# embedded-software-laboratory/p-dmpc

Hardware: AMD Instinct MI355X
Metric: MPC steps/sec (whole node) + p50 per-step plan latency, N vehicles H=8 (higher is better)
Workload: dtype f64

## Files before the change

include/pdmpc.h:

```cpp
#ifndef PDMPC_H
#define PDMPC_H

#include <stddef.h>
#include <stdint.h>

#ifdef __cplusplus
extern "C" {
#endif

#define PDMPC_HP_MAX 16
#define PDMPC_VMAX 8
#define PDMPC_JOINT_MAX 4

enum {
    PDMPC_OK = 0,
    PDMPC_EXHAUSTED = 1,
    PDMPC_ARENA_OVERFLOW = 2,
    PDMPC_ERR_INVALID = -1,
    PDMPC_ERR_NO_DEVICE = -2,
    PDMPC_ERR_HIP = -3,
    PDMPC_ERR_CAPACITY = -4,
    PDMPC_ERR_NO_MPA = -5
};

// ... 114 lines not shown
    uint32_t bk_near_key, bk_near_id, bk_ready, bk_hist, bk_misc, bk_pshape, reach_shared, bk_reach, reach;
    uint32_t ints, succ, heap_key, heap_id;
    const char* kernel;
} pdmpc_launch_plan;
int pdmpc_launch_plan_host(const char* tuning, const pdmpc_launch_query* query, pdmpc_launch_plan* plan);

int pdmpc_get_config(pdmpc_handle* handle, pdmpc_config* config, int32_t* mpa_uploaded);

int pdmpc_upload_mpa(pdmpc_handle* handle, const pdmpc_mpa* mpa);
int pdmpc_mpa_reach_host(const pdmpc_mpa* mpa, double* dmax, double* amax);
int pdmpc_reach_lists_host(int32_t Hp, double dmax, double amax, double root_x, double root_y, const double* x, const double* y, const int32_t* step_first,
                           const int32_t* step_count, int32_t* list_offset, int32_t* list);
int pdmpc_mpa_reach_rects_host(const pdmpc_mpa* mpa, int32_t Hp, double* rects);
int pdmpc_reach_lists_oriented_host(int32_t Hp, int32_t n_trims, const double* rects, int32_t root_trim, double root_x, double root_y, double root_yaw, const double* x, const double* y,
                                    const int32_t* step_first, const int32_t* step_count, int32_t* list_offset, int32_t* list);

int pdmpc_plan_batch(pdmpc_handle* handle, int32_t n_vehicles, const pdmpc_vehicle_in* in,
                     pdmpc_vehicle_out* out);

int pdmpc_set_arena_limit(pdmpc_handle* handle, int32_t max_nodes_limit);
int pdmpc_grow_arena(pdmpc_handle* handle, int32_t max_nodes);
int pdmpc_arena_nodes(pdmpc_handle* handle, int32_t* max_nodes, int64_t* regrows);

int pdmpc_plan_step(pdmpc_handle* handle, int32_t n_vehicles, const pdmpc_vehicle_in* in, const int32_t* pred_offset,
                    const int32_t* pred_index, const pdmpc_polygon_set* fallback_shapes, pdmpc_vehicle_out* out);

int pdmpc_plan_step_literal(pdmpc_handle* handle, int32_t n_vehicles, const pdmpc_vehicle_in* in, const int32_t* pred_offset, const int32_t* pred_index,
                            const pdmpc_polygon_set* fallback_shapes, pdmpc_vehicle_out* out);

int pdmpc_pack_batch(pdmpc_handle* handle, int32_t n_vehicles, const pdmpc_vehicle_in* in);
// ... 44 lines not shown

int pdmpc_debug_pop_trace(pdmpc_handle* handle, int32_t vehicle, int32_t capacity, int32_t* ids, int32_t* n);
int pdmpc_debug_tree(pdmpc_handle* handle, int32_t vehicle, int32_t capacity, double* x, double* y,
                     double* yaw, double* g, double* h, int32_t* trim, int32_t* k, int32_t* parent,
                     int32_t* n);

int pdmpc_debug_edge_check(pdmpc_handle* handle, int32_t mode, int32_t n_cases, const int32_t* a_off, const double* a_x, const double* a_y,
                           const int32_t* b_off, const double* b_x, const double* b_y, int32_t* hit);
int pdmpc_debug_interx_soups(pdmpc_handle* handle, int32_t n_cases, const int32_t* a_off, const double* a_x, const double* a_y, const double* b_x,
                             const double* b_y, const int32_t* s_off, const double* s_x, const double* s_y, int32_t* hit);
int pdmpc_debug_sincos(pdmpc_handle* handle, int32_t n, const double* x, double* s, double* c);

int pdmpc_debug_raw_tree(pdmpc_handle* handle, int32_t vehicle, int32_t capacity, double* x, double* y, double* yaw, double* g,
                         double* h, int32_t* trim, int32_t* k, int32_t* parent, double* key, uint8_t* validity, int32_t* n);

int pdmpc_debug_counters(pdmpc_handle* handle, uint64_t* out16);
int pdmpc_debug_packed_offsets(pdmpc_handle* handle, int32_t vehicle, int32_t* lit_off, int32_t* hdv_off, int32_t* ll2);

int pdmpc_debug_progress(pdmpc_handle* handle, int32_t vehicle, uint32_t* words16);

int pdmpc_debug_heap_script(pdmpc_handle* handle, int32_t n, const int32_t* op, const int32_t* id, const double* key,
                            int32_t lds_entries, int32_t* popped, int32_t* n_popped, double* cycles_per_pop,
                            double* cycles_per_push);

int pdmpc_plan_batch_sampled(pdmpc_handle* handle, int32_t n_vehicles, const pdmpc_vehicle_in* in, const uint32_t* seeds,
                             pdmpc_vehicle_out* out);
int pdmpc_plan_step_sampled(pdmpc_handle* handle, int32_t n_vehicles, const pdmpc_vehicle_in* in, const int32_t* pred_offset,
                            const int32_t* pred_index, const pdmpc_polygon_set* fallback_shapes, const uint32_t* seeds,
                            pdmpc_vehicle_out* out);
int pdmpc_set_step_seeds(pdmpc_handle* handle, int32_t n_vehicles, const uint32_t* seeds);
int pdmpc_debug_random_numbers(pdmpc_handle* handle, int32_t count, const uint32_t* seeds, int32_t n, double* out);
// ... 240 lines not shown
```

include/pdmpc_reach.h:

```cpp
#ifndef PDMPC_REACH_H
#define PDMPC_REACH_H

#include <math.h>

#include "pdmpc_math.h"

#define PDMPC_REACH_FINITE 0x1p64
#define PDMPC_REACH_MARGIN 0x1p-20

PDMPC_HD static inline double pdmpc_reach_radius(double dmax, double amax, int k) {
    const double r = (double)(k - 1) * dmax + amax;
    return r + r * 0x1p-50;
}

PDMPC_HD static inline void pdmpc_reach_box(double dmax, double amax, int k, double root_x, double root_y, double* box) {
    const double R = pdmpc_reach_radius(dmax, amax, k);
    const double rho = R + PDMPC_REACH_MARGIN * (1.0 + fabs(root_x) + fabs(root_y) + R);
    box[0] = root_x - rho;
    box[1] = root_x + rho;
    box[2] = root_y - rho;
    box[3] = root_y + rho;
}

PDMPC_HD static inline int pdmpc_reach_in(double x0, double y0, double x1, double y1, double x_lo, double x_hi, double y_lo, double y_hi) {
// ... 19 lines not shown

PDMPC_HD static inline int pdmpc_reach_in_oriented(double x0, double y0, double x1, double y1, double root_x, double root_y, double cs, double sn, double x_lo, double x_hi, double y_lo,
                                                   double y_hi) {
    if (x0 != x0 || y0 != y0 || x1 != x1 || y1 != y1) return 0;
    const int bounded = fabs(x0) <= PDMPC_REACH_FINITE && fabs(y0) <= PDMPC_REACH_FINITE && fabs(x1) <= PDMPC_REACH_FINITE && fabs(y1) <= PDMPC_REACH_FINITE;
    if (!bounded) return 1;
    const double dx0 = x0 - root_x, dy0 = y0 - root_y, dx1 = x1 - root_x, dy1 = y1 - root_y;
    const double u0 = cs * dx0 + sn * dy0, v0 = cs * dy0 - sn * dx0;
    const double u1 = cs * dx1 + sn * dy1, v1 = cs * dy1 - sn * dx1;
    const double slack = PDMPC_REACH_ROTATION * (fabs(dx0) + fabs(dy0) + fabs(dx1) + fabs(dy1));
    const double max_u = u0 > u1 ? u0 : u1, min_u = u0 < u1 ? u0 : u1;
    const double max_v = v0 > v1 ? v0 : v1, min_v = v0 < v1 ? v0 : v1;
    return !(max_u < x_lo - slack || min_u > x_hi + slack || max_v < y_lo - slack || min_v > y_hi + slack);
}

#endif
```

p-dmpc_amd/csrc/api.cpp:

```cpp
#include <hip/hip_runtime.h>

#include <algorithm>
#include <cmath>
#include <cstdio>
#include <cstdlib>
#include <chrono>
#include <cstring>
#include <limits>
#include <mutex>
#include <string>
#include <type_traits>
#include <vector>

#include "choice_host.hpp"
#include "handle.hpp"
#include "mpa_reach.hpp"
#include "reference_tree.hpp"

namespace {

thread_local std::string g_err;

int failed(int rc, const std::string& err) { return rc ? fail(rc, err) : PDMPC_OK; }

// ... 206 lines not shown
    {
        std::string err;
        if (!parse_tuning(getenv("PDMPC_TUNING"), h->tune, err)) {
            delete h;
            return fail(PDMPC_ERR_INVALID, err);
        }
    }
    h->n_cu = prop.multiProcessorCount > 0 ? prop.multiProcessorCount : 256;
    const uint32_t want_nodes = config->max_nodes > 0 ? (uint32_t)config->max_nodes : 32768u;
    h->max_vehicles = config->max_vehicles > 0 ? config->max_vehicles : 256;
    if (hipStreamCreateWithFlags(&h->stream, hipStreamNonBlocking) != hipSuccess) {
        delete h;
        return fail(PDMPC_ERR_HIP, "hipStreamCreate failed");
    }
    int bad = h->arena.alloc(h->max_vehicles, want_nodes, h->cfg.Hp);
    bad |= h->d_out.ensure((size_t)h->max_vehicles) | h->d_flag.ensure((size_t)h->max_vehicles) | h->d_tree_size.ensure((size_t)h->max_vehicles) | h->d_tie_count.ensure(4) | h->d_work_count.ensure(16);
    bad |= h->d_help_board.ensure((size_t)h->max_vehicles * PDMPC_HB_WORDS) | h->d_help_verdict.ensure((size_t)h->max_vehicles * PDMPC_HELP_CAP) | h->d_help_finished.ensure(16);
    bad |= h->d_bk_post.ensure((size_t)h->max_vehicles * (size_t)h->tune.ready * 6);
    if (bad) {
        delete h;
        return fail(PDMPC_ERR_HIP, "hipMalloc failed for the per-vehicle arenas (lower max_nodes / max_vehicles)");
    }
    (void)hipMemsetAsync(h->d_flag.p, 0, h->d_flag.cap * sizeof(uint32_t), h->stream);
    (void)hipMemsetAsync(h->d_tree_size.p, 0, h->d_tree_size.cap * sizeof(int32_t), h->stream);
    (void)hipMemsetAsync(h->d_tie_count.p, 0, 4 * sizeof(int32_t), h->stream);
    (void)hipMemsetAsync(h->d_work_count.p, 0, 16 * sizeof(unsigned long long), h->stream);
    (void)hipMemsetAsync(h->d_out.p, 0, h->d_out.cap * sizeof(pdmpc_vehicle_out), h->stream);
    (void)hipStreamSynchronize(h->stream);
    *out_handle = h;
    return PDMPC_OK;
}

int pdmpc_launch_plan_host(const char* tuning, const pdmpc_launch_query* q, pdmpc_launch_plan* plan) {
    if (!q || !plan) return fail(PDMPC_ERR_INVALID, "pdmpc_launch_plan_host: null argument");
    if (q->kind < kPlanSearch || q->kind > kPlanJoint) return fail(PDMPC_ERR_INVALID, "pdmpc_launch_plan_host: unknown kind");
    std::string err;
    return failed(plan_query(tuning, *q, *plan, err), err);
}

int pdmpc_sampled_plan_host(const char* tuning, const pdmpc_launch_query* q, int32_t n_expansions_max, pdmpc_launch_plan* plan, int64_t* extra) {
    if (!q || !plan || !extra) return fail(PDMPC_ERR_INVALID, "pdmpc_sampled_plan_host: null argument");
// ... 96 lines not shown
}

int pdmpc_mpa_reach_rects_host(const pdmpc_mpa* mpa, int32_t Hp, double* rects) {
    if (!mpa || !rects || !mpa->transition || !mpa->maneuver_index || (mpa->n_maneuvers > 0 && !mpa->maneuvers)) return fail(PDMPC_ERR_INVALID, "pdmpc_mpa_reach_rects_host: null argument");
    if (mpa->n_trims < 1 || Hp < 1 || Hp > PDMPC_HP_MAX || Hp > mpa->Hp) return fail(PDMPC_ERR_INVALID, "pdmpc_mpa_reach_rects_host: Hp out of range");
    mpa_reach_rects(mpa, Hp, rects);
    return PDMPC_OK;
}

int pdmpc_reach_lists_oriented_host(int32_t Hp, int32_t n_trims, const double* rects, int32_t root_trim, double root_x, double root_y, double root_yaw, const double* x, const double* y,
                                    const int32_t* step_first, const int32_t* step_count, int32_t* list_offset, int32_t* list) {
    if (Hp < 1 || Hp > PDMPC_HP_MAX || !rects || root_trim < 1 || root_trim > n_trims || !step_first || !step_count || !list_offset)
        return fail(PDMPC_ERR_INVALID, "pdmpc_reach_lists_oriented_host: bad argument");
    std::string err;
    return failed(reach_lists_oriented(Hp, rects, root_trim, root_x, root_y, root_yaw, x, y, step_first, step_count, list_offset, list, err), err);
}

int pdmpc_upload_mpa(pdmpc_handle* h, const pdmpc_mpa* mpa) {
    if (!h || !mpa) return fail(PDMPC_ERR_INVALID, "null argument");
    if (mpa->n_trims < 1 || mpa->n_trims > 1023) return fail(PDMPC_ERR_INVALID, "n_trims must be in 1..1023");
    if (mpa->Hp < h->cfg.Hp) return fail(PDMPC_ERR_INVALID, "mpa.Hp smaller than config.Hp");
    if (!mpa->transition || !mpa->maneuver_index || (mpa->n_maneuvers > 0 && !mpa->maneuvers)) return fail(PDMPC_ERR_INVALID, "null table");
    ON_DEVICE(h->cfg.device);
    const int n = mpa->n_trims, Hp = h->cfg.Hp;
    LaunchDims sizes{h->cfg.checker, Hp, n};
    mpa_table_sizes(sizes);
    const int nw = sizes.n_words;
    std::vector<uint64_t> mask((size_t)Hp * n * nw + 2, 0);
    for (int k = 0; k < Hp; ++k)
        for (int i = 0; i < n; ++i)
            for (int j = 0; j < n; ++j)
                if (mpa->transition[((size_t)k * n + i) * n + j]) {
                    const int mi = mpa->maneuver_index[i * n + j];
                    if (mi < 0 || mi >= mpa->n_maneuvers) return fail(PDMPC_ERR_INVALID, "transition allowed but maneuver missing");
                    mask[((size_t)k * n + i) * nw + j / 64] |= 1ull << (j % 64);
                }
    std::vector<int16_t> mi((size_t)n * n + 8, -1);
    for (int i = 0; i < n * n; ++i) mi[i] = (int16_t)mpa->maneuver_index[i];
    const int T = mpa->n_maneuvers;
    std::vector<DevManPose> pose((size_t)std::max(T, 1));
    std::vector<double> area((size_t)std::max(T, 1) * 3 * PDMPC_VMAX * 2 + 2 + (size_t)n * Hp * 4, 0.0);
    for (int t = 0; t < T; ++t) {
        const pdmpc_maneuver& m = mpa->maneuvers[t];
        if (m.n_cols < 2 || m.n_cols > PDMPC_VMAX) return fail(PDMPC_ERR_INVALID, "maneuver area column count out of range");
        pose[t].dx = m.dx;
        pose[t].dy = m.dy;
        pose[t].dyaw = m.dyaw;
        pose[t].n_cols = m.n_cols;
        pose[t].pad = 0;
        const double(*src[3])[PDMPC_VMAX] = {m.area, m.area_without_offset, m.area_large_offset};
        for (int a = 0; a < 3; ++a)
            for (int v = 0; v < m.n_cols; ++v) {
                area[(((size_t)t * 3 + a) * PDMPC_VMAX + v) * 2 + 0] = src[a][0][v];
                area[(((size_t)t * 3 + a) * PDMPC_VMAX + v) * 2 + 1] = src[a][1][v];
            }
    }
    mpa_reach(mpa, area[(size_t)T * 3 * PDMPC_VMAX * 2], area[(size_t)T * 3 * PDMPC_VMAX * 2 + 1]);
    mpa_reach_rects(mpa, Hp, &area[(size_t)T * 3 * PDMPC_VMAX * 2 + 2]);
    if (h->d_mask.ensure(mask.size()) || h->d_mi.ensure(mi.size()) || h->d_pose.ensure(pose.size()) || h->d_area.ensure(area.size()))
        return fail(PDMPC_ERR_HIP, "hipMalloc failed for the MPA tables");
    HIPCHK(hipMemcpy(h->d_mask.p, mask.data(), mask.size() * 8, hipMemcpyHostToDevice));
    HIPCHK(hipMemcpy(h->d_mi.p, mi.data(), mi.size() * 2, hipMemcpyHostToDevice));
    HIPCHK(hipMemcpy(h->d_pose.p, pose.data(), pose.size() * sizeof(DevManPose), hipMemcpyHostToDevice));
    HIPCHK(hipMemcpy(h->d_area.p, area.data(), area.size() * 8, hipMemcpyHostToDevice));
    h->n_trims = n;
    h->n_words = nw;
    h->n_man = T;
    h->mask_bytes = sizes.mask_bytes;
    h->mi_bytes = sizes.mi_bytes;
    h->mpa_alg_bytes = (int64_t)8 * T * (3 + 6 * PDMPC_VMAX) + (int64_t)n * n * Hp / 8;
    h->has_mpa = true;
    return PDMPC_OK;
}
// ... 48 lines not shown

int pdmpc_select_bank(pdmpc_handle* h, int32_t bank) {
    if (!h) return fail(PDMPC_ERR_INVALID, "null handle");
    if (bank < 0 || bank >= 4096) return fail(PDMPC_ERR_INVALID, "bank out of range");
    if ((size_t)bank >= h->banks.size()) h->banks.resize((size_t)bank + 1);
    h->bank = bank;
    return PDMPC_OK;
}

int pdmpc_reset_stats(pdmpc_handle* h) {
    if (!h) return fail(PDMPC_ERR_INVALID, "null handle");
    ON_DEVICE(h->cfg.device);
    HIPCHK(hipStreamSynchronize(h->stream));
    h->timer.reset();
    HIPCHK(hipMemsetAsync(h->d_tie_count.p, 0, 4 * sizeof(int32_t), h->stream));
    HIPCHK(hipMemsetAsync(h->d_work_count.p, 0, 16 * sizeof(unsigned long long), h->stream));
    return PDMPC_OK;
}

int pdmpc_launch_range(pdmpc_handle* h, int32_t first, int32_t count) {
    if (!h) return fail(PDMPC_ERR_INVALID, "null handle");
    ON_DEVICE(h->cfg.device);
    return launch_range(h, first, count, h->safe_launches);
}

int pdmpc_synchronize(pdmpc_handle* h) {
    if (!h) return fail(PDMPC_ERR_INVALID, "null handle");
    ON_DEVICE(h->cfg.device);
    HIPCHK(sync_stream(h));
    return PDMPC_OK;
}
// ... 539 lines not shown

int pdmpc_export_results_async(pdmpc_handle* h, int32_t first, int32_t n, void* dev_records) {
    if (!h || (n > 0 && !dev_records)) return fail(PDMPC_ERR_INVALID, "null argument");
    if (int rc = check_result_slots(h, first, n)) return rc;
    ON_DEVICE(h->cfg.device);
    if (n > 0) HIPCHK(hipMemcpyAsync(dev_records, h->d_out.p + first, (size_t)n * sizeof(pdmpc_vehicle_out), hipMemcpyDeviceToDevice, h->stream));
    return PDMPC_OK;
}

int pdmpc_stream(pdmpc_handle* h, void** hip_stream) {
    if (!h || !hip_stream) return fail(PDMPC_ERR_INVALID, "null argument");
    *hip_stream = (void*)h->stream;
    return PDMPC_OK;
}

int pdmpc_debug_counters(pdmpc_handle* h, uint64_t* out16) {
    if (!h || !out16) return fail(PDMPC_ERR_INVALID, "null argument");
    ON_DEVICE(h->cfg.device);
    HIPCHK(hipStreamSynchronize(h->stream));
    HIPCHK(hipMemcpy(out16, h->d_work_count.p, 16 * sizeof(unsigned long long), hipMemcpyDeviceToHost));
    return PDMPC_OK;
}

int pdmpc_debug_packed_offsets(pdmpc_handle* h, int32_t vehicle, int32_t* lit_off, int32_t* hdv_off, int32_t* ll2) {
    if (!h || !lit_off || !hdv_off || !ll2) return fail(PDMPC_ERR_INVALID, "null argument");
    const PackedStep& B = h->banks[h->bank];
    if (B.pack_failed || vehicle < 0 || vehicle >= B.n_packed) return fail(PDMPC_ERR_INVALID, "pdmpc_debug_packed_offsets: no such vehicle in the packed batch");
    const DevVehicle& d = B.host.veh[B.inv.empty() ? vehicle : B.inv[(size_t)vehicle]];
    for (int k = 0; k <= h->cfg.Hp; ++k) {
        lit_off[k] = d.lit_off[k];
        hdv_off[k] = d.hdv_off[k];
    }
    ll2[0] = d.ll_off;
    ll2[1] = d.ll_len;
    return PDMPC_OK;
// ... 256 lines not shown
```

p-dmpc_amd/csrc/bulk_search.hpp:

```cpp
#include <hip/hip_runtime.h>

#include "search_common.hpp"

#include "frontier_common.hpp"

#include "bk_shared.hpp"
#include "bk_helper.hpp"

#define BK_P2 3
#define BK_PER PDMPC_BK_PER
#define BK_FAST_PER 4

namespace {

__device__ __forceinline__ unsigned long long wg_scan_excl(unsigned long long v, lds_vu64* wsum, int lane, int wave, int n_waves, unsigned long long& total) {
    unsigned long long inc = v;
#pragma unroll
    for (int o = 1; o < PDMPC_WAVE; o <<= 1) {
        const unsigned long long t = __shfl_up(inc, o);
        inc += lane >= o ? t : 0ull;
    }
    if (lane == PDMPC_WAVE - 1) wsum[wave] = inc;
    __syncthreads();
    unsigned long long off = 0, tot = 0;
// ... 53 lines not shown
            int cols = 0;
            while (cols < PDMPC_VMAX && !is_nan(poly[cols].x)) ++cols;
            hit = cols > 0 && sat_pair_lane(pt, ncols, poly, cols);
        }
#pragma unroll 1
        for (int j = 0; CHECKER == PDMPC_CHECK_INTERX && j + 1 < PDMPC_VMAX; ++j) {
            asm volatile("" : "+v"(pt[0].x), "+v"(pt[0].y), "+v"(pt[1].x), "+v"(pt[1].y), "+v"(pt[2].x), "+v"(pt[2].y), "+v"(pt[3].x), "+v"(pt[3].y), "+v"(pt[4].x), "+v"(pt[4].y),
                         "+v"(pt[5].x), "+v"(pt[5].y), "+v"(pt[6].x), "+v"(pt[6].y), "+v"(pt[7].x), "+v"(pt[7].y));
            const d2 q1 = poly[j + 1];
            hit = hit || interx_segment_n<PDMPC_VMAX>(pt, ncols - 1, q0, q1);
            q0 = q1;
        }
        if (hit) {
            vs_store(VS, i0, VS_INVALID);
            atomicOr((uint32_t*)&sh[FR_FLAGS], FRF_INVALIDATED);
        }
    }
}

#define BK_NB 256
__device__ __forceinline__ uint32_t bk_bin(double key, double lo, double scale) {
    const double t = (key - lo) * scale;
    if (!(t > 0.0)) return 0u;
    return t < (double)(BK_NB - 1) ? (uint32_t)t : (uint32_t)(BK_NB - 1);
}
__device__ __forceinline__ void bk_select(const lds_u32* bins, uint32_t target, int lane, uint32_t& bin, uint32_t& cum) {
    uint32_t hq[4];
#pragma unroll
    for (int q = 0; q < 4; ++q) hq[q] = bins[4 * lane + q];
    const uint32_t loc = hq[0] + hq[1] + hq[2] + hq[3];
// ... 1048 lines not shown
        }
        BK_TICK2(0)
        if (verify_req) {
            verify_req = false;
            const unsigned long long arr = sh_load64(sh, BK_FD_LO);
            uint32_t nn = sh[FR_NNODES];
            nn = nn < S.max_nodes ? nn : S.max_nodes;
            uint32_t items = 0;
            for (int k = 0; k < Hp; ++k)
                items += (vcnt[k] < A.max_nodes ? vcnt[k] : A.max_nodes) * (uint32_t)__builtin_popcountll(chg[k] & arr);
            if (ticking) {
                unsigned long long due = 0;
                for (int k = 0; k < Hp; ++k) due += (unsigned long long)__builtin_popcountll(chg[k] & arr);
                atomicAdd(A.work_count + 14, due);
                atomicAdd(A.work_count + 15, (unsigned long long)(Hp * __builtin_popcountll(arr)));
            }
            BK_TICK2(5)
            bk_recheck_items<CHECKER>(S, VS, CK, P, BK_VLIST(1), vcnt, A.max_nodes, items, arr, chg, sh, tid, bd);
            __syncthreads();
            BK_TICK2(1)
            flags = sh[FR_FLAGS];
            bool best_alive = false;
            if ((flags & FRF_INVALIDATED) && sh[FR_BEST_ID] != 0u) {
                const uint32_t g = sh[FR_BEST_ID];
                double b1;
                best_alive = vs_load(VS, g - 1u) == VS_VALID && fr_goal_path(S, VS, F.gkey, g, b1);
            }
            const bool lost_best = (flags & FRF_INVALIDATED) && !best_alive;
            const bool reopen = lost_best && sh[FR_DROPPED] != 0u;
            const uint32_t n_parked = sh[BK_NTENT];
            if (n_parked) {
                const bool fits = sh[FR_NEAR_N] + n_parked <= OC;
                const double l_far = sh_ld_d(sh, FR_L_FAR);
// ... 6 lines not shown
                    if (tent) vs_store(VS, i0, VS_UNKNOWN);
                    const bool push = tent && !reopen;
                    to_near(push && fits && !(k > l_far), k, i0 + 1u);
                    to_far(push && !(fits && !(k > l_far)), k, i0 + 1u);
                }
            }
            BK_TICK2(2)
            if (flags & FRF_INVALIDATED) {
                pb_valid = false;
                rec_valid = false;
            }
            vs_copied = false;
            __syncthreads();
            if (tid == 0) {
                sh[BK_ARRIVALS] = sh[BK_ARRIVALS] + 1u;
                sh[BK_FD_LO] = 0;
                sh[BK_FD_HI] = 0;
                for (int k = 0; k < Hp; ++k) chg[k] = 0ull;
                sh[BK_NTENT] = 0;
                sh_st_d(sh, BK_TENT_MIN, inf);
                if (flags & FRF_INVALIDATED) {
                    sh[FR_EVER_INVAL] = 1;
                    if (lost_best) {
                        sh[FR_BEST_ID] = 0;
                        sh[FR_PATH_FOR] = 0;
                    }
                    sh[FR_FLAGS] = flags & ~FRF_INVALIDATED;
                }
                if (reopen) {
                    sh[FR_NEAR_N] = 0;
// ... 681 lines not shown
```

p-dmpc_amd/csrc/lds_layout.hpp:

```cpp
#pragma once
#include <cstddef>

#define SH_WORD_TABLE(X)                                                                                                                  \
    X(SH_STATE, 0, 32)        \
                                                                                                                          \
    X(SH_NNODES, 3, 32)            \
                                                                                                                             \
    X(SH_PEND_LO, 5, 32)      \
    X(SH_PEND_HI, 6, 32)                                                                                                                  \
    X(SH_ARR_LO, 7, 32)                \
    X(SH_ARR_HI, 8, 32)                                                                                                                   \
                                                                                                                             \
    X(BK_MID_N, 10, 32)                                                                           \
    X(BK_MID_PAD, 11, 32)                                       \
    X(BK_MID_MIN, 12, 64)                                                            \
    X(BK_L_MID, 14, 64)       \
    X(BK_FD_LO, 16, 32)       \
    X(BK_FD_HI, 17, 32)       \
    X(BK_WAITRES, 18, 32)     \
    X(BK_PUBLISHED, 19, 32)   \
    X(BK_TIEMODE, 20, 32)     \
    X(BK_RP_NEED, 21, 32)                \
    X(BK_RP_GOAL, 22, 32)                                               \
    X(BK_RP_NPOP, 23, 32)                                                                                           \
// ... 73 lines not shown
struct BkMisc {
    uint32_t gp_path[32];
    double gp_mp[32];
    unsigned long long wsum64[32];
    uint32_t wsum[32];
    uint32_t chm[8];
    unsigned long long tk[12];
    uint32_t ref_ids[PDMPC_HP_MAX + 2];
    unsigned long long tk2[7];
    uint32_t bins[256];
};
static_assert(sizeof(BkMisc) == 2048, "PDMPC_LKX_PSHAPE puts the next region 2048 bytes behind PDMPC_LKX_MISC");
static_assert(offsetof(BkMisc, bins) == 1024, "the selection's histogram is the second KB of the region");
static_assert(offsetof(BkMisc, tk) % 8 == 0 && offsetof(BkMisc, tk2) % 8 == 0 && offsetof(BkMisc, tk2) == offsetof(BkMisc, ref_ids) + sizeof(BkMisc::ref_ids), "no padding between the tables");

struct BkHist {
    uint32_t goal_list[1024];
    uint32_t vlist[1024];
    uint32_t voffs[1024];
};
static_assert(sizeof(BkHist) == 3072 * 4, "PDMPC_LKX_MISC puts the next region 3072 words behind PDMPC_LKX_HIST");

namespace {

typedef LDS_AS unsigned long long lds_u64s;

__device__ __forceinline__ LDS_AS BkMisc* bk_misc(LDS_AS unsigned char* lsm) { return (LDS_AS BkMisc*)(lsm + PDMPC_LK_MISC); }
__device__ __forceinline__ LDS_AS BkHist* bk_hist(LDS_AS unsigned char* lsm) { return (LDS_AS BkHist*)(lsm + PDMPC_LK_HIST); }

}

#define BK_PSHAPE(lsm) ((lds_d2*)((lsm) + PDMPC_LK_PSHAPE))
#define BK_PCOLS(pshape, Hp) ((lds_u32*)((pshape) + (Hp) * PDMPC_VMAX))
#define BK_PCHG(pshape, Hp) ((lds_u64s*)(BK_PCOLS(pshape, Hp) + PDMPC_HP_MAX))
#define BK_PVCNT(pshape, Hp) ((lds_u32*)(BK_PCHG(pshape, Hp) + PDMPC_HP_MAX))
```

p-dmpc_amd/csrc/mpa_reach.hpp:

```cpp
#pragma once
#include <algorithm>
#include <cmath>
#include <cstring>
#include <limits>
#include <map>
#include <string>
#include <utility>
#include <vector>

#include "../../include/pdmpc.h"
#include "../../include/pdmpc_math.h"
#include "../../include/pdmpc_reach.h"

inline void mpa_reach(const pdmpc_mpa* mpa, double& dmax, double& amax) {
    dmax = 0.0;
    amax = 0.0;
    for (int t = 0; t < mpa->n_maneuvers; ++t) {
        const pdmpc_maneuver& m = mpa->maneuvers[t];
        dmax = std::max(dmax, hypot(m.dx, m.dy));
        const double(*src[3])[PDMPC_VMAX] = {m.area, m.area_without_offset, m.area_large_offset};
        for (int a = 0; a < 3; ++a)
            for (int v = 0; v < m.n_cols && v < PDMPC_VMAX; ++v) amax = std::max(amax, hypot(src[a][0][v], src[a][1][v]));
    }
}

typedef std::pair<double, double> ReachPt;
inline void reach_hull(std::vector<ReachPt>& P, std::vector<ReachPt>& H) {
    std::sort(P.begin(), P.end());
    P.erase(std::unique(P.begin(), P.end()), P.end());
    const size_t n = P.size();
    if (n < 3) return;
    auto cross = [](const ReachPt& o, const ReachPt& a, const ReachPt& b) { return (a.first - o.first) * (b.second - o.second) - (a.second - o.second) * (b.first - o.first); };
    H.clear();
    for (size_t i = 0; i < n; ++i) {
        while (H.size() >= 2 && cross(H[H.size() - 2], H.back(), P[i]) <= 0) H.pop_back();
        H.push_back(P[i]);
    }
// ... 114 lines not shown
```

p-dmpc_amd/pdmpc/backend.py:

```python
import ctypes as C
import math
import os

import numpy as np

from . import abi
from .abi import ChoiceStruct, FcaGroup
from .prototypes import PROTOTYPES, declare

_HERE = os.path.dirname(os.path.abspath(__file__))
LIB_PATH = os.environ.get("PDMPC_LIB") or os.path.join(os.path.dirname(_HERE), "csrc", "libpdmpc_hip.so")

_LIB = None

EXPORTS = list(PROTOTYPES)
SAMPLED_BUDGET_DEFAULT, SAMPLED_BUDGET_MAX = 250, 16384
SAMPLED_ENSEMBLE_MAX, SAMPLED_ENSEMBLE_STRIDE = 16, 1000003
_SAMPLED_EXTRA = ("node_cap", "tree_in_lds", "tree_hbm_bytes", "rand_chunk", "member_bytes", "ensemble_tree_bytes", "grid", "n_members")


def sampled_member_seed(seed, member):
    return int(load_library().pdmpc_sampled_member_seed(int(seed) & 0xFFFFFFFF, int(member)))


# ... 995 lines not shown
        ao, ax, ay = _flat_columns(a_list)
        _, bx, by = _flat_columns(b_list)
        so, sx, sy = _flat_columns([s for t in soups for s in t])
        hit = np.zeros(max(n, 1), dtype=np.int32)
        rc = self.L.pdmpc_debug_interx_soups(self.h, n, abi.i32p(ao), abi.dp(ax), abi.dp(ay), abi.dp(bx), abi.dp(by), abi.i32p(so), abi.dp(sx), abi.dp(sy), abi.i32p(hit))
        _check(self.L, rc, "pdmpc_debug_interx_soups")
        return hit[:n].copy()

    def debug_sincos(self, x):
        x = np.ascontiguousarray(x, dtype=np.float64).ravel()
        s, c = np.zeros_like(x), np.zeros_like(x)
        _check(self.L, self.L.pdmpc_debug_sincos(self.h, x.size, abi.dp(x), abi.dp(s), abi.dp(c)), "pdmpc_debug_sincos")
        return s, c

    def debug_counters(self):
        out = (C.c_uint64 * 16)()
        _check(self.L, self.L.pdmpc_debug_counters(self.h, out), "pdmpc_debug_counters")
        return list(out)

    def progress(self, vehicle):
        w = (C.c_uint32 * 32)()
        _check(self.L, self.L.pdmpc_debug_progress(self.h, vehicle, w), "pdmpc_debug_progress")
        return list(w)

    def tree(self, vehicle, capacity=1 << 16):
        f = {k: np.zeros(capacity) for k in ("x", "y", "yaw", "g", "h")}
        i = {k: np.zeros(capacity, dtype=np.int32) for k in ("trim", "k", "parent")}
        n = C.c_int32()
        args = [abi.dp(f[k]) for k in ("x", "y", "yaw", "g", "h")] + [abi.i32p(i[k]) for k in ("trim", "k", "parent")]
        _check(self.L, self.L.pdmpc_debug_tree(self.h, vehicle, capacity, *args, C.byref(n)), "pdmpc_debug_tree")
        nn = min(n.value, capacity)
# ... 4 lines not shown
```

p-dmpc_amd/pdmpc/prototypes.py:

```python
import ctypes as C

from . import abi

P = C.POINTER
INT, STR = C.c_int, C.c_char_p
OBJ = C.c_void_p
VOIDP = C.c_void_p
I32, I64, U32, F64 = C.c_int32, C.c_int64, C.c_uint32, C.c_double
DP, IP, BP, UP = abi.c_double_p, abi.c_int32_p, abi.c_uint8_p, abi.c_uint32_p
CONFIG, MPA, POLYS, VIN, VOUT, CHOICE = P(abi.Config), P(abi.Mpa), P(abi.PolygonSet), P(abi.VehicleIn), P(abi.VehicleOut), P(abi.ChoiceStruct)

STEP = [I32, VIN, IP, IP, POLYS]
STEP_OUT = [P(I32), P(VIN), P(IP), P(IP), P(POLYS)]
POSES = [DP, DP, DP, DP, IP]
TABLE = [I32, I32, POLYS]
COUPLED = [BP, DP]
BOUND = POSES + [POLYS, I32, I32, IP, DP, DP, BP]
FCA = [I32, I32, DP, DP, DP, DP, I32, IP, POLYS, POLYS, F64, F64, F64, IP, IP]
FCA_GROUPED = [I32, P(abi.FcaGroup), I32, DP, DP, DP, DP, IP, IP]
CHOSEN = [CHOICE, IP, DP]
UNIQUE = [I32, BP, I64, P(I64), UP, IP]
UNIQUE_GROUPED = [I32, IP, P(BP), P(I64), P(I64), UP, IP]

PROTOTYPES = {
    "pdmpc_create": (INT, [CONFIG, P(OBJ)]),
    "pdmpc_destroy": (INT, [OBJ]),
    "pdmpc_launch_plan_host": (INT, [STR, P(abi.LaunchQuery), P(abi.LaunchPlan)]),
    "pdmpc_get_config": (INT, [OBJ, CONFIG, P(I32)]),
    "pdmpc_upload_mpa": (INT, [OBJ, MPA]),
    "pdmpc_mpa_reach_host": (INT, [MPA, DP, DP]),
    "pdmpc_reach_lists_host": (INT, [I32, F64, F64, F64, F64, DP, DP, IP, IP, IP, IP]),
    "pdmpc_mpa_reach_rects_host": (INT, [MPA, I32, DP]),
    "pdmpc_reach_lists_oriented_host": (INT, [I32, I32, DP, I32, F64, F64, F64, DP, DP, IP, IP, IP, IP]),
    "pdmpc_plan_batch": (INT, [OBJ, I32, VIN, VOUT]),
    "pdmpc_set_arena_limit": (INT, [OBJ, I32]),
    "pdmpc_grow_arena": (INT, [OBJ, I32]),
    "pdmpc_arena_nodes": (INT, [OBJ, P(I32), P(I64)]),
    "pdmpc_plan_step": (INT, [OBJ] + STEP + [VOUT]),
    "pdmpc_plan_step_literal": (INT, [OBJ] + STEP + [VOUT]),
    "pdmpc_pack_batch": (INT, [OBJ, I32, VIN]),
    "pdmpc_plan_step_lean": (INT, [OBJ] + STEP + [IP, DP]),
    "pdmpc_fetch_records_at": (INT, [OBJ, I32, IP, VOUT]),
    "pdmpc_choose_host": (INT, [I32, IP, DP] + CHOSEN),
    "pdmpc_choose_resident": (INT, [OBJ, I32] + CHOSEN + [VOUT]),
    "pdmpc_plan_step_chosen": (INT, [OBJ] + STEP + CHOSEN + [VOUT]),
    "pdmpc_choice_kernel_ms": (INT, [OBJ, DP]),
    "pdmpc_last_call_timing": (INT, [OBJ, DP]),
    "pdmpc_launch_packed": (INT, [OBJ]),
# ... 165 lines not shown
```

Before: 1631.

## Cull bulk re-check items with bounding circles before exact polygon intersection

Each maneuver's swept area now gets a precomputed bounding circle, stored after the reach rectangles in the MPA area table. In the bulk search's interx re-check, every (node, polygon) item is first tested cheaply: the circle is transformed by the parent pose and compared against the polygon's bounding box. Only survivors are compacted into an LDS list in tiles and given the full segment-intersection test. This adds a decode pass, extra block syncs per tile and two debug counters, in exchange for skipping the exact test on items that are clearly disjoint.

```diff
diff --git a/include/pdmpc.h b/include/pdmpc.h
--- a/include/pdmpc.h
+++ b/include/pdmpc.h
@@ -152,6 +152,9 @@
 int pdmpc_mpa_reach_rects_host(const pdmpc_mpa* mpa, int32_t Hp, double* rects);
 int pdmpc_reach_lists_oriented_host(int32_t Hp, int32_t n_trims, const double* rects, int32_t root_trim, double root_x, double root_y, double root_yaw, const double* x, const double* y,
                                     const int32_t* step_first, const int32_t* step_count, int32_t* list_offset, int32_t* list);
+
+int pdmpc_mpa_area_circles_host(const pdmpc_mpa* mpa, double* circles);
+int pdmpc_recheck_out_host(double cx, double cy, double r, double cs, double sn, double px, double py, const double* x, const double* y, int32_t n_cols);
 
 int pdmpc_plan_batch(pdmpc_handle* handle, int32_t n_vehicles, const pdmpc_vehicle_in* in,
                      pdmpc_vehicle_out* out);
@@ -226,7 +229,8 @@
 int pdmpc_debug_raw_tree(pdmpc_handle* handle, int32_t vehicle, int32_t capacity, double* x, double* y, double* yaw, double* g,
                          double* h, int32_t* trim, int32_t* k, int32_t* parent, double* key, uint8_t* validity, int32_t* n);
 
-int pdmpc_debug_counters(pdmpc_handle* handle, uint64_t* out16);
+#define PDMPC_DEBUG_COUNTERS 18
+int pdmpc_debug_counters(pdmpc_handle* handle, uint64_t* out);
 int pdmpc_debug_packed_offsets(pdmpc_handle* handle, int32_t vehicle, int32_t* lit_off, int32_t* hdv_off, int32_t* ll2);
 
 int pdmpc_debug_progress(pdmpc_handle* handle, int32_t vehicle, uint32_t* words16);
diff --git a/include/pdmpc_reach.h b/include/pdmpc_reach.h
--- a/include/pdmpc_reach.h
+++ b/include/pdmpc_reach.h
@@ -57,4 +57,24 @@
     return !(max_u < x_lo - slack || min_u > x_hi + slack || max_v < y_lo - slack || min_v > y_hi + slack);
 }
 
+PDMPC_HD static inline int pdmpc_recheck_out(double cx, double cy, double r, double cs, double sn, double px, double py, const double* qx, const double* qy, int n_cols) {
+    const double wx = cs * cx - sn * cy + px, wy = sn * cx + cs * cy + py;
+    const double rho = r + PDMPC_REACH_MARGIN * (1.0 + fabs(px) + fabs(py) + r);
+    double x_lo = HUGE_VAL, x_hi = -HUGE_VAL, y_lo = HUGE_VAL, y_hi = -HUGE_VAL;
+    int real = 0, wild = 0;
+    for (int i = 0; i < n_cols; ++i) {
+        const double x = qx[i], y = qy[i];
+        const int ok = x == x && y == y;
+        wild |= ok && !(fabs(x) <= PDMPC_REACH_FINITE && fabs(y) <= PDMPC_REACH_FINITE);
+        real += ok;
+        x_lo = ok && x < x_lo ? x : x_lo;
+        x_hi = ok && x > x_hi ? x : x_hi;
+        y_lo = ok && y < y_lo ? y : y_lo;
+        y_hi = ok && y > y_hi ? y : y_hi;
+    }
+    if (real < 2) return 1;
+    if (wild || !(fabs(wx) <= PDMPC_REACH_FINITE) || !(fabs(wy) <= PDMPC_REACH_FINITE) || !(rho <= PDMPC_REACH_FINITE)) return 0;
+    return wx + rho < x_lo || wx - rho > x_hi || wy + rho < y_lo || wy - rho > y_hi;
+}
+
 #endif
diff --git a/p-dmpc_amd/csrc/api.cpp b/p-dmpc_amd/csrc/api.cpp
--- a/p-dmpc_amd/csrc/api.cpp
+++ b/p-dmpc_amd/csrc/api.cpp
@@ -244,7 +244,7 @@
         return fail(PDMPC_ERR_HIP, "hipStreamCreate failed");
     }
     int bad = h->arena.alloc(h->max_vehicles, want_nodes, h->cfg.Hp);
-    bad |= h->d_out.ensure((size_t)h->max_vehicles) | h->d_flag.ensure((size_t)h->max_vehicles) | h->d_tree_size.ensure((size_t)h->max_vehicles) | h->d_tie_count.ensure(4) | h->d_work_count.ensure(16);
+    bad |= h->d_out.ensure((size_t)h->max_vehicles) | h->d_flag.ensure((size_t)h->max_vehicles) | h->d_tree_size.ensure((size_t)h->max_vehicles) | h->d_tie_count.ensure(4) | h->d_work_count.ensure(PDMPC_DEBUG_COUNTERS);
     bad |= h->d_help_board.ensure((size_t)h->max_vehicles * PDMPC_HB_WORDS) | h->d_help_verdict.ensure((size_t)h->max_vehicles * PDMPC_HELP_CAP) | h->d_help_finished.ensure(16);
     bad |= h->d_bk_post.ensure((size_t)h->max_vehicles * (size_t)h->tune.ready * 6);
     if (bad) {
@@ -254,7 +254,7 @@
     (void)hipMemsetAsync(h->d_flag.p, 0, h->d_flag.cap * sizeof(uint32_t), h->stream);
     (void)hipMemsetAsync(h->d_tree_size.p, 0, h->d_tree_size.cap * sizeof(int32_t), h->stream);
     (void)hipMemsetAsync(h->d_tie_count.p, 0, 4 * sizeof(int32_t), h->stream);
-    (void)hipMemsetAsync(h->d_work_count.p, 0, 16 * sizeof(unsigned long long), h->stream);
+    (void)hipMemsetAsync(h->d_work_count.p, 0, PDMPC_DEBUG_COUNTERS * sizeof(unsigned long long), h->stream);
     (void)hipMemsetAsync(h->d_out.p, 0, h->d_out.cap * sizeof(pdmpc_vehicle_out), h->stream);
     (void)hipStreamSynchronize(h->stream);
     *out_handle = h;
@@ -381,6 +381,17 @@
         return fail(PDMPC_ERR_INVALID, "pdmpc_reach_lists_oriented_host: bad argument");
     std::string err;
     return failed(reach_lists_oriented(Hp, rects, root_trim, root_x, root_y, root_yaw, x, y, step_first, step_count, list_offset, list, err), err);
+}
+
+int pdmpc_mpa_area_circles_host(const pdmpc_mpa* mpa, double* circles) {
+    if (!mpa || !circles || (mpa->n_maneuvers > 0 && !mpa->maneuvers)) return fail(PDMPC_ERR_INVALID, "pdmpc_mpa_area_circles_host: null argument");
+    mpa_area_circles(mpa, circles);
+    return PDMPC_OK;
+}
+
+int pdmpc_recheck_out_host(double cx, double cy, double r, double cs, double sn, double px, double py, const double* x, const double* y, int32_t n_cols) {
+    if (n_cols < 0 || (n_cols > 0 && (!x || !y))) return fail(PDMPC_ERR_INVALID, "pdmpc_recheck_out_host: bad argument");
+    return pdmpc_recheck_out(cx, cy, r, cs, sn, px, py, x, y, n_cols);
 }
 
 int pdmpc_upload_mpa(pdmpc_handle* h, const pdmpc_mpa* mpa) {
@@ -406,7 +417,7 @@
     for (int i = 0; i < n * n; ++i) mi[i] = (int16_t)mpa->maneuver_index[i];
     const int T = mpa->n_maneuvers;
     std::vector<DevManPose> pose((size_t)std::max(T, 1));
-    std::vector<double> area((size_t)std::max(T, 1) * 3 * PDMPC_VMAX * 2 + 2 + (size_t)n * Hp * 4, 0.0);
+    std::vector<double> area((size_t)std::max(T, 1) * 3 * PDMPC_VMAX * 2 + 2 + (size_t)n * Hp * 4 + (size_t)std::max(T, 1) * 3, 0.0);
     for (int t = 0; t < T; ++t) {
         const pdmpc_maneuver& m = mpa->maneuvers[t];
         if (m.n_cols < 2 || m.n_cols > PDMPC_VMAX) return fail(PDMPC_ERR_INVALID, "maneuver area column count out of range");
@@ -424,6 +435,7 @@
     }
     mpa_reach(mpa, area[(size_t)T * 3 * PDMPC_VMAX * 2], area[(size_t)T * 3 * PDMPC_VMAX * 2 + 1]);
     mpa_reach_rects(mpa, Hp, &area[(size_t)T * 3 * PDMPC_VMAX * 2 + 2]);
+    mpa_area_circles(mpa, &area[(size_t)T * 3 * PDMPC_VMAX * 2 + 2 + (size_t)n * Hp * 4]);
     if (h->d_mask.ensure(mask.size()) || h->d_mi.ensure(mi.size()) || h->d_pose.ensure(pose.size()) || h->d_area.ensure(area.size()))
         return fail(PDMPC_ERR_HIP, "hipMalloc failed for the MPA tables");
     HIPCHK(hipMemcpy(h->d_mask.p, mask.data(), mask.size() * 8, hipMemcpyHostToDevice));
@@ -502,7 +514,7 @@
     HIPCHK(hipStreamSynchronize(h->stream));
     h->timer.reset();
     HIPCHK(hipMemsetAsync(h->d_tie_count.p, 0, 4 * sizeof(int32_t), h->stream));
-    HIPCHK(hipMemsetAsync(h->d_work_count.p, 0, 16 * sizeof(unsigned long long), h->stream));
+    HIPCHK(hipMemsetAsync(h->d_work_count.p, 0, PDMPC_DEBUG_COUNTERS * sizeof(unsigned long long), h->stream));
     return PDMPC_OK;
 }
 
@@ -1072,11 +1084,11 @@
     return PDMPC_OK;
 }
 
-int pdmpc_debug_counters(pdmpc_handle* h, uint64_t* out16) {
-    if (!h || !out16) return fail(PDMPC_ERR_INVALID, "null argument");
+int pdmpc_debug_counters(pdmpc_handle* h, uint64_t* out) {
+    if (!h || !out) return fail(PDMPC_ERR_INVALID, "null argument");
     ON_DEVICE(h->cfg.device);
     HIPCHK(hipStreamSynchronize(h->stream));
-    HIPCHK(hipMemcpy(out16, h->d_work_count.p, 16 * sizeof(unsigned long long), hipMemcpyDeviceToHost));
+    HIPCHK(hipMemcpy(out, h->d_work_count.p, PDMPC_DEBUG_COUNTERS * sizeof(unsigned long long), hipMemcpyDeviceToHost));
     return PDMPC_OK;
 }
 
diff --git a/p-dmpc_amd/csrc/bulk_search.hpp b/p-dmpc_amd/csrc/bulk_search.hpp
--- a/p-dmpc_amd/csrc/bulk_search.hpp
+++ b/p-dmpc_amd/csrc/bulk_search.hpp
@@ -91,6 +91,135 @@
         if (hit) {
             vs_store(VS, i0, VS_INVALID);
             atomicOr((uint32_t*)&sh[FR_FLAGS], FRF_INVALIDATED);
+        }
+    }
+}
+
+struct BkRcItem {
+    uint32_t i0, a;
+    int ks;
+};
+__device__ __forceinline__ BkRcItem bk_rc_decode(uint32_t item, int Hp, const uint32_t* vlist, const lds_u32* vcnt, uint32_t cap, unsigned long long arr, const lds_u64s* chg) {
+    uint32_t v = item, n_k = 1;
+    int ks = 1;
+    bool found = false;
+    for (int q = 1; q <= Hp; ++q) {
+        const uint32_t nq = vcnt[q - 1] < cap ? vcnt[q - 1] : cap;
+        const uint32_t m = nq * (uint32_t)__builtin_popcountll(chg[q - 1] & arr);
+        const bool here = !found && v < m;
+        ks = here ? q : ks;
+        n_k = here ? nq : n_k;
+        found = found || here;
+        v -= found ? 0u : m;
+    }
+    v = found ? v : 0u;
+    BkRcItem r;
+    r.a = v / n_k;
+    r.i0 = vlist[(size_t)(ks - 1) * cap + (v - r.a * n_k)];
+    r.ks = ks;
+    return r;
+}
+__device__ __forceinline__ int nth_bit_wave(unsigned long long mask, uint32_t rk) {
+    for (uint32_t b = 0; __ballot(b < rk) != 0ull; ++b) mask = b < rk ? mask & (mask - 1ull) : mask;
+    return mask ? (int)__builtin_ctzll(mask) : 0;
+}
+
+__device__ __forceinline__ void bk_recheck_culled(const KernelArgs& A, const Search& S, const VState& VS, const BkCheck& C, const SpecCtx& P, const uint32_t* vlist, const lds_u32* vcnt, uint32_t cap,
+                                                  uint32_t items, unsigned long long arr, const lds_u64s* chg, volatile lds_u32* sh, lds_u32* list, int tid, int nthreads, bool counting) {
+    const int lane = tid & (PDMPC_WAVE - 1);
+    const uint32_t w0 = (uint32_t)(tid - lane);
+    int turn = 0;
+    for (uint32_t base = 0; base < items; base += BK_RC_TILE, turn ^= 1) {
+        if (base) __syncthreads();
+        const uint32_t end = items - base < BK_RC_TILE ? items : base + BK_RC_TILE;
+        const int cw = turn ? BK_RC_N1 : BK_RC_N0;
+        for (uint32_t t0 = base + w0; t0 < end; t0 += (uint32_t)nthreads) {
+            const BkItemCtx I = bk_item_ctx<PDMPC_CHECK_INTERX>(C);
+            const bool in = t0 + (uint32_t)lane < end;
+            const uint32_t item = in ? t0 + (uint32_t)lane : t0;
+            const BkRcItem it = bk_rc_decode(item, I.Hp(), vlist, vcnt, cap, arr, chg);
+            uint32_t parent, packed;
+            piece_link(node_piece(S, it.i0, 3), parent, packed);
+            const unsigned long long due = chg[it.ks - 1] & arr;
+            const bool live = in && vs_load(VS, it.i0) == VS_VALID && parent != 0u && it.a < (uint32_t)__builtin_popcountll(due);
+            const uint32_t pi = parent ? parent - 1u : 0u;
+            const int m = live ? NODE_MAN(packed) : 0;
+            const int p = nth_bit_wave(due, live ? it.a : 0u);
+            const d2 pxy = node_piece(S, pi, 0), pcs = node_piece(S, pi, 2);
+            const int cb = A.n_man * (3 * PDMPC_VMAX * 2) + 2 + A.n_trims * A.Hp * 4 + 3 * m;
+            const double ccx = A.man_area[cb], ccy = A.man_area[cb + 1], cr = A.man_area[cb + 2];
+            const lds_d2* poly = I.l_soup() + P.l_soff[it.ks - 1] + P.l_lit[it.ks - 1] + p * PDMPC_VMAX;
+            double qx[PDMPC_VMAX], qy[PDMPC_VMAX];
+#pragma unroll
+            for (int i = 0; i < PDMPC_VMAX; ++i) {
+                const d2 q = poly[i];
+                qx[i] = q.x;
+                qy[i] = q.y;
+            }
+            const bool keep = live && !pdmpc_recheck_out(ccx, ccy, cr, pcs.x, pcs.y, pxy.x, pxy.y, qx, qy, PDMPC_VMAX);
+            const unsigned long long bm = __ballot(keep);
+            if (bm) {
+                const uint32_t at = sh_add_uniform(sh, cw, (uint32_t)__builtin_popcountll(bm), lane) + lane_rank(bm, lane);
+                if (keep && at < BK_RC_TILE) list[at] = item;
+                if (keep && at >= BK_RC_TILE) atomicOr((uint32_t*)&sh[FR_FLAGS], FRF_BUG);
+            }
+        }
+        __syncthreads();
+        uint32_t n = sh[cw];
+        n = n < BK_RC_TILE ? n : BK_RC_TILE;
+        if (tid == 0) {
+            sh[turn ? BK_RC_N0 : BK_RC_N1] = 0u;
+            if (counting) atomicAdd(A.work_count + 17, (unsigned long long)n);
+        }
+        for (uint32_t e0 = w0; e0 < n; e0 += (uint32_t)nthreads) {
+            const BkItemCtx I = bk_item_ctx<PDMPC_CHECK_INTERX>(C);
+            const bool have = e0 + (uint32_t)lane < n;
+            const uint32_t item = list[have ? e0 + (uint32_t)lane : e0];
+            const BkRcItem it = bk_rc_decode(item, I.Hp(), vlist, vcnt, cap, arr, chg);
+            const uint32_t i0 = it.i0;
+            uint32_t parent, packed;
+            piece_link(node_piece(S, i0, 3), parent, packed);
+            const int k = it.ks, m = NODE_MAN(packed), ncols = NODE_COLS(packed);
+            const int p = nth_bit_wave(chg[k - 1] & arr, it.a);
+            const uint32_t pi = parent ? parent - 1u : 0u;
+            const d2 pxy = node_piece(S, pi, 0), pcs = node_piece(S, pi, 2);
+            const double cc = pcs.x, ss = pcs.y, pX = pxy.x, pY = pxy.y;
+            const size_t abase = (size_t)m * 3 * PDMPC_VMAX;
+            d2 pt[PDMPC_VMAX];
+            if (C.areas_in_lds) {
+#pragma unroll
+                for (int i = 0; i < PDMPC_VMAX; ++i) pt[i] = I.l_area()[abase + i];
+            } else {
+#pragma unroll
+                for (int i = 0; i < PDMPC_VMAX; ++i) pt[i] = C.g_area[abase + i];
+            }
+#pragma unroll
+            for (int i = 0; i < PDMPC_VMAX; ++i) {
+                const d2 ar = pt[i];
+                pt[i].x = cc * ar.x - ss * ar.y + pX;
+                pt[i].y = ss * ar.x + cc * ar.y + pY;
+            }
+            const lds_d2* poly = I.l_soup() + P.l_soff[k - 1] + P.l_lit[k - 1] + p * PDMPC_VMAX;
+            int last = 0;
+#pragma unroll
+            for (int j = 1; j < PDMPC_VMAX; ++j) {
+                const d2 q = poly[j];
+                last = (q.x == q.x && q.y == q.y) ? j : last;
+            }
+            d2 q0 = poly[0];
+            bool hit = false;
+#pragma unroll 1
+            for (int j = 0; j + 1 < PDMPC_VMAX && __ballot(j < last) != 0ull; ++j) {
+                asm volatile("" : "+v"(pt[0].x), "+v"(pt[0].y), "+v"(pt[1].x), "+v"(pt[1].y), "+v"(pt[2].x), "+v"(pt[2].y), "+v"(pt[3].x), "+v"(pt[3].y), "+v"(pt[4].x), "+v"(pt[4].y),
+                             "+v"(pt[5].x), "+v"(pt[5].y), "+v"(pt[6].x), "+v"(pt[6].y), "+v"(pt[7].x), "+v"(pt[7].y));
+                const d2 q1 = poly[j + 1];
+                hit = hit || interx_segment_n<PDMPC_VMAX>(pt, ncols - 1, q0, q1);
+                q0 = q1;
+            }
+            if (hit && have) {
+                vs_store(VS, i0, VS_INVALID);
+                atomicOr((uint32_t*)&sh[FR_FLAGS], FRF_INVALIDATED);
+            }
         }
     }
 }
@@ -1169,9 +1298,13 @@
                 for (int k = 0; k < Hp; ++k) due += (unsigned long long)__builtin_popcountll(chg[k] & arr);
                 atomicAdd(A.work_count + 14, due);
                 atomicAdd(A.work_count + 15, (unsigned long long)(Hp * __builtin_popcountll(arr)));
+                if (CHECKER == PDMPC_CHECK_INTERX) atomicAdd(A.work_count + 16, (unsigned long long)items);
             }
             BK_TICK2(5)
-            bk_recheck_items<CHECKER>(S, VS, CK, P, BK_VLIST(1), vcnt, A.max_nodes, items, arr, chg, sh, tid, bd);
+            if (CHECKER == PDMPC_CHECK_INTERX)
+                bk_recheck_culled(A, S, VS, CK, P, BK_VLIST(1), vcnt, A.max_nodes, items, arr, chg, sh, hist, tid, bd, ticking);
+            else
+                bk_recheck_items<CHECKER>(S, VS, CK, P, BK_VLIST(1), vcnt, A.max_nodes, items, arr, chg, sh, tid, bd);
             __syncthreads();
             BK_TICK2(1)
             flags = sh[FR_FLAGS];
@@ -1208,6 +1341,8 @@
             __syncthreads();
             if (tid == 0) {
                 sh[BK_ARRIVALS] = sh[BK_ARRIVALS] + 1u;
+                sh[BK_RC_N0] = 0u;
+                sh[BK_RC_N1] = 0u;
                 sh[BK_FD_LO] = 0;
                 sh[BK_FD_HI] = 0;
                 for (int k = 0; k < Hp; ++k) chg[k] = 0ull;
diff --git a/p-dmpc_amd/csrc/lds_layout.hpp b/p-dmpc_amd/csrc/lds_layout.hpp
--- a/p-dmpc_amd/csrc/lds_layout.hpp
+++ b/p-dmpc_amd/csrc/lds_layout.hpp
@@ -3,7 +3,8 @@
 
 #define SH_WORD_TABLE(X)                                                                                                                  \
     X(SH_STATE, 0, 32)        \
-                                                                                                                          \
+    X(BK_RC_N0, 1, 32)        \
+    X(BK_RC_N1, 2, 32)                                                                                                                    \
     X(SH_NNODES, 3, 32)            \
                                                                                                                              \
     X(SH_PEND_LO, 5, 32)      \
@@ -111,12 +112,14 @@
 static_assert(offsetof(BkMisc, bins) == 1024, "the selection's histogram is the second KB of the region");
 static_assert(offsetof(BkMisc, tk) % 8 == 0 && offsetof(BkMisc, tk2) % 8 == 0 && offsetof(BkMisc, tk2) == offsetof(BkMisc, ref_ids) + sizeof(BkMisc::ref_ids), "no padding between the tables");
 
+#define BK_RC_TILE 3072u
 struct BkHist {
     uint32_t goal_list[1024];
     uint32_t vlist[1024];
     uint32_t voffs[1024];
 };
 static_assert(sizeof(BkHist) == 3072 * 4, "PDMPC_LKX_MISC puts the next region 3072 words behind PDMPC_LKX_HIST");
+static_assert(sizeof(BkHist) == BK_RC_TILE * 4, "the survivors' list of a tile of the re-check cull fills the region");
 
 namespace {
 
diff --git a/p-dmpc_amd/csrc/mpa_reach.hpp b/p-dmpc_amd/csrc/mpa_reach.hpp
--- a/p-dmpc_amd/csrc/mpa_reach.hpp
+++ b/p-dmpc_amd/csrc/mpa_reach.hpp
@@ -21,6 +21,34 @@
         const double(*src[3])[PDMPC_VMAX] = {m.area, m.area_without_offset, m.area_large_offset};
         for (int a = 0; a < 3; ++a)
             for (int v = 0; v < m.n_cols && v < PDMPC_VMAX; ++v) amax = std::max(amax, hypot(src[a][0][v], src[a][1][v]));
+    }
+}
+
+inline void mpa_area_circles(const pdmpc_mpa* mpa, double* circles) {
+    double dmax, amax;
+    mpa_reach(mpa, dmax, amax);
+    for (int t = 0; t < mpa->n_maneuvers; ++t) {
+        const pdmpc_maneuver& m = mpa->maneuvers[t];
+        const int n = std::min((int)m.n_cols, (int)PDMPC_VMAX);
+        double x_lo = 0.0, x_hi = 0.0, y_lo = 0.0, y_hi = 0.0;
+        for (int v = 0; v < n; ++v) {
+            const double x = m.area[0][v], y = m.area[1][v];
+            x_lo = v == 0 || x < x_lo ? x : x_lo;
+            x_hi = v == 0 || x > x_hi ? x : x_hi;
+            y_lo = v == 0 || y < y_lo ? y : y_lo;
+            y_hi = v == 0 || y > y_hi ? y : y_hi;
+        }
+        double cx = 0.5 * x_lo + 0.5 * x_hi, cy = 0.5 * y_lo + 0.5 * y_hi, r = 0.0;
+        for (int v = 0; v < n; ++v) r = std::max(r, hypot(m.area[0][v] - cx, m.area[1][v] - cy));
+        r = r + r * 0x1p-40;
+        if (!(r <= PDMPC_REACH_FINITE) || !(fabs(cx) + fabs(cy) <= 0x1p20 * (1.0 + r))) {
+            cx = 0.0;
+            cy = 0.0;
+            r = amax + amax * 0x1p-40;
+        }
+        circles[3 * t] = cx;
+        circles[3 * t + 1] = cy;
+        circles[3 * t + 2] = r;
     }
 }
 
diff --git a/p-dmpc_amd/pdmpc/backend.py b/p-dmpc_amd/pdmpc/backend.py
--- a/p-dmpc_amd/pdmpc/backend.py
+++ b/p-dmpc_amd/pdmpc/backend.py
@@ -1033,7 +1033,7 @@
         return s, c
 
     def debug_counters(self):
-        out = (C.c_uint64 * 16)()
+        out = (C.c_uint64 * 18)()
         _check(self.L, self.L.pdmpc_debug_counters(self.h, out), "pdmpc_debug_counters")
         return list(out)
 
diff --git a/p-dmpc_amd/pdmpc/prototypes.py b/p-dmpc_amd/pdmpc/prototypes.py
--- a/p-dmpc_amd/pdmpc/prototypes.py
+++ b/p-dmpc_amd/pdmpc/prototypes.py
@@ -32,6 +32,8 @@
     "pdmpc_reach_lists_host": (INT, [I32, F64, F64, F64, F64, DP, DP, IP, IP, IP, IP]),
     "pdmpc_mpa_reach_rects_host": (INT, [MPA, I32, DP]),
     "pdmpc_reach_lists_oriented_host": (INT, [I32, I32, DP, I32, F64, F64, F64, DP, DP, IP, IP, IP, IP]),
+    "pdmpc_mpa_area_circles_host": (INT, [MPA, DP]),
+    "pdmpc_recheck_out_host": (INT, [F64, F64, F64, F64, F64, F64, F64, DP, DP, I32]),
     "pdmpc_plan_batch": (INT, [OBJ, I32, VIN, VOUT]),
     "pdmpc_set_arena_limit": (INT, [OBJ, I32]),
     "pdmpc_grow_arena": (INT, [OBJ, I32]),
```

Measured after the change: 1627. No clear change (-0.2%).
